# srihari-humbarwadi/retinanet-tensorflow2.x

Hardware: AMD Instinct MI355X
Metric: images/sec train, ResNet50-640 RetinaNet data-parallel step (encode + fwd + loss + bwd + clip + all-reduce + SGD/EMA); inference images/s under `infer` (higher is better)
Workload: dtype bf16; 1 GPU; ResNet50-640x640 bf16 training, 32 images/GPU (BASELINE configs[2] shard: global batch 32), resnet_initial frozen, single GPU; global_batch=32, parallelism=dp1, rccl_ranks=1, comm=torch, syncbn_messages=0

## Files before the change

### include/rnet_hip.h

```cpp
#ifndef RNET_HIP_H_
#define RNET_HIP_H_

#include <stddef.h>
#include <stdint.h>

#ifdef __cplusplus
extern "C" {
#endif
#if defined(__GNUC__)
#pragma GCC visibility push(default)
#endif

typedef enum {
  RN_OK = 0,
  RN_EINVAL = -1,
  RN_ENOMEM = -2,
  RN_EHIP = -3,
  RN_ECOMM = -4,
  RN_EUNSUPPORTED = -5
} rn_status;

enum { RN_DT_F32 = 0, RN_DT_BF16 = 1 };
enum { RN_ACT_NONE = 0, RN_ACT_RELU = 1, RN_ACT_RELU6 = 2, RN_ACT_SWISH = 3 };

// ... 67 lines not shown
  int32_t wgrad_target_blocks;
  int32_t ablate;
  int32_t splitk_target_blocks;
} rn_launch_opts;

typedef struct rn_handle rn_handle;
int rn_create(int device_id, rn_handle** out);
int rn_destroy(rn_handle* h);
int rn_handle_device(const rn_handle* h);
int rn_handle_num_cus(const rn_handle* h);
int rn_handle_set_launch_opts(rn_handle* h, const rn_launch_opts* opts);
int rn_handle_get_launch_opts(const rn_handle* h, rn_launch_opts* opts);
int rn_handle_comm_init(rn_handle* h, int slot, const void* unique_id , int rank, int world);
void* rn_handle_comm(const rn_handle* h, int slot);
int rn_handle_comm_destroy(rn_handle* h, int slot);

#define RN_CONV_MAX_SEGMENTS 10

typedef struct {
  const void* x;
  const void* w;
  void* y;
  const float* scale;
  const float* shift;
  const void* residual;
  int32_t N, H, W, Cin, pix_stride, Ho, Wo, Cout;
  float* bn_partial;
  const float* bias;
  int32_t w_terms;
  int32_t w_pair;
  const void* bn_bwd_y;
  const float* bn_bwd_fwd;
} rn_conv_segment;

typedef struct {
  int32_t R, S, stride_h, stride_w, pad_top, pad_left;
  int32_t act;
  int32_t out_dtype;
  int32_t num_segments;
  rn_conv_segment seg[RN_CONV_MAX_SEGMENTS];
  rn_launch_opts opts;
  void* splitk_ws;
  int64_t splitk_ws_bytes;
} rn_conv_problem;

int rn_conv2d_nhwc_fwd(const rn_conv_problem* problem , void* stream);
size_t rn_conv_splitk_workspace_bytes(const rn_conv_problem* problem );
size_t rn_conv_splitk_workspace_max_bytes(void);

int rn_conv_cout_pad(int Cout);
int rn_conv_tile_rows(const rn_conv_problem* problem);
int rn_conv_bn_row_blocks(const rn_conv_problem* problem, int segment);
int rn_conv_kernel_id(const rn_conv_problem* problem);
int rn_conv_cin_pad(int Cin);
int rn_pack_conv_weight(const float* w_hwio, int R, int S, int Cin, int Cout, int Cin_pad, void* w_packed,
                        void* stream);
int rn_pack_conv_weight_split(const float* w, int layout_ohwi, int R, int S, int Cin, int Cout, int Cin_pad, int terms,
                              void* w_packed, void* stream);
int rn_conv_pair_rows(int Cout);
int rn_pack_conv_weight_pair(const float* w, int layout_ohwi, int R, int S, int Cin, int Cout, int Cin_pad,
                             void* w_packed, void* stream);
int rn_pack_conv_weight_ohwi(const float* w_ohwi, int R, int S, int Cin, int Cout, int Cin_pad, void* w_packed,
                             void* stream);
int rn_pack_stem_weight(const float* w_hwio, int Cout, void* w_packed, void* stream);
int rn_stem_padded_width(int W);
int rn_pack_stem_input(const float* images, int N, int H, int W, void* packed, void* stream);
int rn_pack_stem_weight_rs(const float* w_hwio, int R, int S, int Cout, void* w_packed, void* stream);
int rn_pack_image_nhwc4(const float* images, int N, int H, int W, int pad_top, int pad_left, int Hp, int Wp,
                        void* packed, void* stream);

typedef struct {
  const void* x;
  const void* dy;
  int32_t N, H, W, Cin, Ho, Wo, Cout;
  int32_t dy_pix_stride;
  int32_t x_pix_stride;
} rn_wgrad_segment;

typedef struct {
  int32_t R, S, stride_h, stride_w, pad_top, pad_left;
  int32_t num_segments;
  rn_wgrad_segment seg[RN_CONV_MAX_SEGMENTS];
  rn_launch_opts opts;
} rn_wgrad_problem;

size_t rn_wgrad_workspace_bytes(const rn_wgrad_problem* problem );
int rn_wgrad_kernel_id(const rn_wgrad_problem* problem );
int rn_conv2d_nhwc_wgrad(const rn_wgrad_problem* problem , float* dw, float beta, void* workspace,
                         size_t workspace_bytes, void* stream);
size_t rn_wgrad_group_workspace_bytes(const rn_wgrad_problem* const* problems , int n);
int rn_wgrad_group_fused(const rn_wgrad_problem* const* problems , int n);
int rn_conv2d_nhwc_wgrad_group(const rn_wgrad_problem* const* problems , int n, float* const* dws ,
                               float beta, void* workspace, size_t workspace_bytes, void* stream);

int rn_pack_conv_weight_dgrad(const float* w_ohwi, int R, int S, int Cin, int Cout, int Cout_pad, void* w_packed,
                              void* stream);
#define RN_DGRAD_PACK_MAX 64
typedef struct {
  const float* w_ohwi;
  void* w_packed;
  int32_t R, S, Cin, Cout, Cout_pad;
  int32_t pad_;
} rn_dgrad_pack;
int rn_pack_conv_weight_dgrad_batch(const rn_dgrad_pack* items , int n, void* stream);
int rn_cast_pad_f32_to_bf16(const float* x, void* y, int64_t P, int C, int Cpad, void* stream);
int rn_reduce_rows_f32(const float* src, int rows, int64_t row_stride, int n, float add, float* dst, void* stream);
// ... 188 lines not shown
```

### retinanet-tensorflow2.x_amd/csrc/rn_conv_dev.h

```cpp
#ifndef RN_CONV_DEV_H_
#define RN_CONV_DEV_H_
#include "rn_common.h"

typedef rn_h16 bf16x8_t __attribute__((ext_vector_type(8)));
typedef float f32x16_t __attribute__((ext_vector_type(16)));

#define CONV_THREADS 256

struct ConvSegDev {
  const uint16_t* x;
  const uint16_t* w;
  void* y;
  const float* scale;
  const float* shift;
  const uint16_t* residual;
  float* bn_partial;
  const float* bias;
  const uint16_t* bn_y;
  const float* bn_fwd;
  int N, H, W, Cin, pix_stride, Ho, Wo, Cout;
  int M, tile_begin, n_tiles, CinP;
  int cwrap, halo_pitch;
  int pair_cout, rows;
};


struct ConvArgs {
  int R, S, sh, sw, pt, pl, act, nseg, total_tiles, pad_;
  int split_f, split_s, vtotal, pad2_;
  float* ws;
  ConvSegDev seg[RN_CONV_MAX_SEGMENTS];
};

#define RN_SPLITK_HEADER_BYTES 16384
#define RN_SPLITK_SLOT_BYTES (256 * 256 * 4)

template <int BK>
__device__ __forceinline__ int lds_swz(int row) {
  constexpr int SLOTS = BK / 8;
  constexpr int RPB = 256 / (BK * 2);
  return (row / RPB) % SLOTS;
}
template <int BK>
__device__ __forceinline__ int lds_slot_off(int row, int slot) {
  return (row * (BK / 8) + (slot ^ lds_swz<BK>(row))) * 16;
}

typedef __attribute__((address_space(3))) void lds_void_t;

__device__ __forceinline__ void dma16(__amdgpu_buffer_rsrc_t rsrc, char* lds_wave_base, unsigned voff) {
  __builtin_amdgcn_raw_ptr_buffer_load_lds(rsrc, (lds_void_t*)lds_wave_base, 16, (int)voff, 0, 0, 0);
}

#define RN_OOB 0x80000000u


int rn_launch_conv128(const ConvArgs& a, int BN, int BK, bool f32, bool split, hipStream_t st);
int rn_launch_conv_big(const ConvArgs& a, bool out_f32, const rn_launch_opts& opts, hipStream_t st);
int rn_launch_conv_halo(const ConvArgs& a, bool out_f32, const rn_launch_opts& opts, hipStream_t st, int wm = 2);
int rn_conv_halo_patch_pixels(int N, int H, int W, int pitch, int BM = 256);
int rn_conv_halo_pitch(int W);
int rn_conv_halo_capacity(int BM = 256);
#endif
```

### retinanet-tensorflow2.x_amd/csrc/rn_conv_dispatch.hip

```cpp
#include <algorithm>
#include <map>
#include <mutex>
#include <tuple>

#include "rn_conv_dev.h"

extern "C" int rn_conv_cout_pad(int Cout) { return Cout <= 64 ? 64 : (int)rn_align_up((size_t)Cout, 128); }
extern "C" int rn_conv_cin_pad(int Cin) { return Cin <= 32 ? 32 : (int)rn_align_up((size_t)Cin, 64); }
extern "C" int rn_conv_pair_rows(int Cout) { return Cout > 0 ? 128 * ((Cout + 63) / 64) : 0; }

struct ConvPlanSeg {
  int cols, cols_pad;
  int terms, cin_pad;
  long long M;
  int n_tiles, tile_begin;
  int bn_row_blocks;
};

struct ConvPlan {
  int kid;
  int BM, BN;
  int BK;
  int bal_rows;
  bool deal;
  bool fast_div;
  int order[RN_CONV_MAX_SEGMENTS];
  long long total_tiles;
  int min_depth;
  int split_parts;
  long long ws_bytes;
  ConvPlanSeg seg[RN_CONV_MAX_SEGMENTS];
};

static long long seg_tiles(const ConvPlanSeg& s, int rows, int width) { return rn_cdiv(s.M, rows) * rn_cdiv(s.cols_pad, width); }
static long long conv_tiles(const ConvPlan& pl, int nseg, int rows, int width) {
  long long t = 0;
  for (int i = 0; i < nseg; ++i) t += seg_tiles(pl.seg[i], rows, width);
  return t;
}

static bool conv_halo_fits(const rn_conv_problem* p, int BM) {
  if (p->opts.conv_no_halo) return false;
  if (p->R != 3 || p->S != 3 || p->stride_h != 1 || p->stride_w != 1 || p->pad_top != 1 || p->pad_left != 1)
    return false;
  static std::mutex mu;
  static std::map<std::tuple<int, int, int, int>, int> patch_px;
  for (int i = 0; i < p->num_segments; ++i) {
    const rn_conv_segment& s = p->seg[i];
    if (s.Ho != s.H || s.Wo != s.W || s.Cin % 32 != 0) return false;
    if ((long long)s.N * s.H * s.W >= (1ll << 22)) return false;
    std::lock_guard<std::mutex> lock(mu);
    const auto key = std::make_tuple(s.N, s.H, s.W, BM);
    auto it = patch_px.find(key);
    if (it == patch_px.end()) it = patch_px.emplace(key, rn_conv_halo_patch_pixels(s.N, s.H, s.W, rn_conv_halo_pitch(s.W), BM)).first;
    if (it->second > rn_conv_halo_capacity(BM)) return false;
  }
  return true;
}

static int splitk_parts(int total, int min_chunks, int G0, long long* bytes) {
  const int L = total % G0;
  if (bytes) *bytes = 0;
  if (L == 0 || L > 511 || min_chunks < 8) return 1;
  int S = G0 / L;
  if (S > min_chunks / 4) S = min_chunks / 4;
  if (S > 4) S = 4;
  if (S < 2) return 1;
  if (bytes) *bytes = RN_SPLITK_HEADER_BYTES + (long long)L * S * RN_SPLITK_SLOT_BYTES;
  return S;
}

static void rn_splitk_plan(ConvArgs& a, int min_chunks, void* ws, long long ws_bytes, const rn_launch_opts& opts) {
  const int total = a.total_tiles;
  a.split_f = total; a.split_s = 1; a.vtotal = total; a.pad2_ = 0; a.ws = nullptr;
  const int G0 = rn_persistent_grid(0x7fffffff, rn_num_cus(), opts);
  const int L = total % G0;
  int S = ws ? splitk_parts(total, min_chunks, G0, nullptr) : 1;
  while (S >= 2 && RN_SPLITK_HEADER_BYTES + (long long)L * S * RN_SPLITK_SLOT_BYTES > ws_bytes) --S;
  if (S < 2) return;
  a.split_f = total - L; a.split_s = S; a.vtotal = L * S; a.ws = (float*)ws;
}

extern "C" size_t rn_conv_splitk_workspace_max_bytes(void) { return RN_SPLITK_HEADER_BYTES + 256ull * RN_SPLITK_SLOT_BYTES; }

static int conv_big_balanced_rows(const rn_conv_problem* p, const ConvPlanSeg& s) {
  if (p->num_segments != 1 || p->R != 1 || p->S != 1 || p->stride_h != 1 || p->stride_w != 1) return 0;
  if (p->opts.conv_tile || p->opts.conv_big_min_tiles || p->opts.max_workgroups || p->splitk_ws) return 0;
  if (s.terms * s.cin_pad > 512) return 0;
  const int n_tiles = (int)rn_cdiv(s.cols_pad, 256);
  const int G = rn_persistent_grid(0x7fffffff, rn_num_cus(), p->opts);
  const long long T = seg_tiles(s, 256, 256);
  if (T <= 0 || G <= 0) return 0;
  const long long rounds = rn_cdiv(T, G);
  const long long m_tiles = rounds * G / n_tiles;
  if (m_tiles < 1) return 0;
  long long rows = rn_cdiv(s.M, m_tiles);
  rows = (rows + 3) / 4 * 4;
  if (rows < 64 || rows > 236) return 0;
  return (int)rows;
}

#define RN_SPLIT128_MIN_STEPS 4
static int conv128_split_parts(const rn_launch_opts& opts, long long tiles, int ksteps, int BN, long long ws_bytes) {
  if (opts.conv_tile == 1 || tiles < 1 || tiles > 4096) return 1;
  const int target = opts.splitk_target_blocks > 0 ? opts.splitk_target_blocks : rn_num_cus() * 3 / 4;
  int S = target / (int)tiles;
  if (S > ksteps / RN_SPLIT128_MIN_STEPS) S = ksteps / RN_SPLIT128_MIN_STEPS;
  if (S > 8) S = 8;
  const long long slot = 128ll * BN * 4;
  while (S >= 2 && RN_SPLITK_HEADER_BYTES + tiles * S * slot > ws_bytes) --S;
  return S >= 2 ? S : 1;
}

static bool conv_plan(const rn_conv_problem* p, bool assume_ws, ConvPlan& pl) {
  if (!p || p->num_segments < 1 || p->num_segments > RN_CONV_MAX_SEGMENTS) return false;
  const int nseg = p->num_segments;
  const rn_launch_opts& o = p->opts;

  bool all_wide = true, all_128 = true, all_128s_or_64 = true, one_col = true;
  bool epi_ok = true;
  long long dmin = 1ll << 60, dmax = 0;
  pl.min_depth = 0x7fffffff;
  pl.fast_div = true;
  for (int i = 0; i < nseg; ++i) {
    const rn_conv_segment& s = p->seg[i];
    ConvPlanSeg& d = pl.seg[i];
    d.cols = s.w_pair ? rn_conv_pair_rows(s.Cout) : s.Cout;
    d.cols_pad = rn_conv_cout_pad(d.cols);
    d.terms = s.w_terms > 1 ? s.w_terms : 1;
    d.cin_pad = rn_conv_cin_pad(s.Cin);
    d.M = (long long)s.N * s.Ho * s.Wo;
    all_wide = all_wide && d.cols_pad >= 256;
    all_128 = all_128 && d.cols_pad == 128;
    all_128s_or_64 = all_128s_or_64 && (d.cols_pad % 128 == 0 || d.cols_pad == 64);
    one_col = one_col && d.cols_pad <= 256;
    epi_ok = epi_ok && s.Cout % (p->out_dtype == RN_DT_F32 && s.w_pair ? 4 : 8) == 0 && !(s.bias && s.residual);
    const int depth = d.terms * d.cin_pad;
    pl.min_depth = depth < pl.min_depth ? depth : pl.min_depth;
    const long long depth_all = (long long)p->R * p->S * d.cin_pad * d.terms;
    dmin = depth_all < dmin ? depth_all : dmin;
    dmax = depth_all > dmax ? depth_all : dmax;
    pl.fast_div = pl.fast_div && d.M < (1 << 22);
  }
  const int cin0 = pl.seg[0].cin_pad;
  pl.BK = (cin0 % 64 != 0 || (long long)p->R * p->S * cin0 <= 256) ? 32 : 64;

  const bool use_big = o.conv_tile != 1 && o.conv_tile != 3 && all_wide && epi_ok &&
                       (o.conv_tile == 2 || conv_tiles(pl, nseg, 256, 256) >= (o.conv_big_min_tiles > 0 ? o.conv_big_min_tiles : 192));
  if (use_big) {
    if (!conv_halo_fits(p, 256)) pl.kid = 1;
    else pl.kid = (o.conv_tile == 0 && o.conv_big_min_tiles == 0 && conv_halo_fits(p, 512)) ? 3 : 2;
  } else {
    const bool halo512 = o.conv_tile != 1 && !o.conv_no_halo && (o.conv_tile == 3 ? all_128s_or_64 : all_128) && epi_ok &&
                         (o.conv_tile >= 2 || conv_tiles(pl, nseg, 512, 128) >= (o.conv_big_min_tiles > 0 ? o.conv_big_min_tiles : 128)) &&
                         conv_halo_fits(p, 512);
    pl.kid = halo512 ? 3 : 0;
  }

  pl.bal_rows = 0;
  if (pl.kid == 0) {
    pl.BM = 128;
    pl.BN = pl.seg[0].cols_pad <= 64 ? 64 : 128;
    if (pl.BN == 128 && o.conv_tile != 1 && 2 * conv_tiles(pl, nseg, 128, 128) <= rn_num_cus()) pl.BN = 64;
  } else if (pl.kid == 3) {
    pl.BM = 512; pl.BN = 128;
  } else {
    pl.BM = 256; pl.BN = 256;
    if (pl.kid == 1) pl.bal_rows = conv_big_balanced_rows(p, pl.seg[0]);
  }

  for (int i = 0; i < nseg; ++i) pl.order[i] = i;
  pl.deal = pl.kid == 1 && nseg > 1 && one_col && dmax >= 2 * dmin;
  if (pl.deal)
    std::stable_sort(pl.order, pl.order + nseg, [&](int x, int y) {
      return pl.seg[x].cin_pad * pl.seg[x].terms > pl.seg[y].cin_pad * pl.seg[y].terms;
    });
  const int rows = pl.bal_rows ? pl.bal_rows : pl.BM;
  pl.total_tiles = 0;
  for (int ii = 0; ii < nseg; ++ii) {
    ConvPlanSeg& d = pl.seg[pl.order[ii]];
    d.n_tiles = (int)rn_cdiv(d.cols_pad, pl.BN);
    d.tile_begin = (int)pl.total_tiles;
    d.bn_row_blocks = (int)(pl.bal_rows ? 2 * rn_cdiv(d.M, rows) : (rows / 128) * rn_cdiv(d.M, rows));
    pl.total_tiles += seg_tiles(d, rows, pl.BN);
  }

  pl.split_parts = 1;
  pl.ws_bytes = 0;
  if (pl.kid == 0) {
    if (p->splitk_ws || assume_ws) {
      const long long avail = p->splitk_ws ? p->splitk_ws_bytes : (long long)rn_conv_splitk_workspace_max_bytes();
      pl.split_parts = conv128_split_parts(o, pl.total_tiles, p->R * p->S * (pl.min_depth / pl.BK), pl.BN, avail);
    }
    if (pl.split_parts >= 2) pl.ws_bytes = RN_SPLITK_HEADER_BYTES + pl.total_tiles * pl.split_parts * 128 * pl.BN * 4;
  } else if (pl.kid == 2) {
    splitk_parts((int)pl.total_tiles, pl.min_depth / 32, rn_persistent_grid(0x7fffffff, rn_num_cus(), o), &pl.ws_bytes);
  }
  return true;
}

extern "C" size_t rn_conv_splitk_workspace_bytes(const rn_conv_problem* p) {
  ConvPlan pl;
  return conv_plan(p, true, pl) ? (size_t)pl.ws_bytes : 0;
}

extern "C" int rn_conv_kernel_id(const rn_conv_problem* p) {
  ConvPlan pl;
  return conv_plan(p, false, pl) ? pl.kid : -1;
}

extern "C" int rn_conv_bn_row_blocks(const rn_conv_problem* p, int segment) {
  ConvPlan pl;
  if (!conv_plan(p, false, pl) || segment < 0 || segment >= p->num_segments) return 0;
  return pl.seg[segment].bn_row_blocks;
}

extern "C" int rn_conv_tile_rows(const rn_conv_problem* p) {
  ConvPlan pl;
  return conv_plan(p, false, pl) ? pl.BM : 0;
}

static int conv_validate(const rn_conv_problem* p, const ConvPlan& pl) {
  RN_CHECK_ARG(p->R >= 1 && p->S >= 1 && p->R * p->S <= 32, "rn_conv2d_nhwc_fwd: R*S=%d > 32", p->R * p->S);
  RN_CHECK_ARG(p->stride_h >= 1 && p->stride_w >= 1, "rn_conv2d_nhwc_fwd: bad stride");
  RN_CHECK_ARG(p->out_dtype == RN_DT_BF16 || p->out_dtype == RN_DT_F32, "rn_conv2d_nhwc_fwd: bad out_dtype");
  if (const int orc = rn_validate_launch_opts(p->opts, "rn_conv2d_nhwc_fwd")) return orc;
  for (int ii = 0; ii < p->num_segments; ++ii) {
    const int i = pl.order[ii];
    const rn_conv_segment& s = p->seg[i];
    RN_CHECK_ARG(s.x && s.w && s.y, "rn_conv2d_nhwc_fwd: segment %d has a null tensor", i);
    RN_CHECK_ARG(s.N > 0 && s.H > 0 && s.W > 0 && s.Ho > 0 && s.Wo > 0 && s.Cout > 0 && s.Cin > 0,
                 "rn_conv2d_nhwc_fwd: segment %d bad shape", i);
    RN_CHECK_ARG(s.Cin % 8 == 0 && pl.seg[i].cin_pad % pl.BK == 0,
                 "rn_conv2d_nhwc_fwd: segment %d Cin=%d must be a multiple of 8 (K step %d)", i, s.Cin, pl.BK);
    RN_CHECK_ARG(s.pix_stride % 4 == 0 && s.pix_stride > 0,
                 "rn_conv2d_nhwc_fwd: segment %d pix_stride=%d must be a positive multiple of 4", i, s.pix_stride);
    RN_CHECK_ARG(s.Cout % 4 == 0, "rn_conv2d_nhwc_fwd: segment %d Cout=%d not a multiple of 4", i, s.Cout);
    RN_CHECK_ARG((pl.seg[i].cols_pad <= 64) == (pl.seg[0].cols_pad <= 64), "rn_conv2d_nhwc_fwd: segments mix Cout tile widths");
    RN_CHECK_ARG(!s.w_pair || (pl.kid != 0 && p->out_dtype == RN_DT_F32 && s.w_terms <= 1 && !s.scale && !s.shift &&
                               !s.residual && !s.bn_partial),
                 "rn_conv2d_nhwc_fwd: segment %d: w_pair needs an f32 launch without scale / shift / residual that the 256- / "
                 "512-row kernels take (rn_conv_kernel_id() != 0)", i);
    RN_CHECK_ARG(((uintptr_t)s.x | (uintptr_t)s.w | (uintptr_t)s.y | (uintptr_t)s.residual) % 16 == 0,
                 "rn_conv2d_nhwc_fwd: segment %d tensors must be 16-byte aligned", i);
    RN_CHECK_ARG(pl.seg[i].M < (1ll << 31) && (long long)s.N * s.H * s.W * s.pix_stride * 2 < (1ll << 31),
                 "rn_conv2d_nhwc_fwd: segment %d input exceeds the 2 GiB buffer-addressing limit", i);
    if (s.bn_bwd_y) {
      RN_CHECK_ARG(s.bn_partial && s.bn_bwd_fwd && p->out_dtype == RN_DT_BF16 && !s.scale && !s.shift && !s.bias &&
                       !s.residual && p->act == RN_ACT_NONE && s.Cout % 8 == 0 && (uintptr_t)s.bn_bwd_y % 16 == 0,
                   "rn_conv2d_nhwc_fwd: segment %d: bn_bwd_y needs bn_partial + bn_bwd_fwd on a plain bf16 launch", i);
    }
    RN_CHECK_ARG((s.bn_bwd_y != nullptr) == (p->seg[0].bn_bwd_y != nullptr),
                 "rn_conv2d_nhwc_fwd: bn_bwd_y must be set on all segments or none");
    RN_CHECK_ARG(pl.seg[i].terms <= 3, "rn_conv2d_nhwc_fwd: segment %d w_terms=%d (1..3)", i, s.w_terms);
  }
  RN_CHECK_ARG(p->splitk_ws == nullptr || ((uintptr_t)p->splitk_ws % 16 == 0 && p->splitk_ws_bytes >= 0),
               "rn_conv2d_nhwc_fwd: splitk_ws must be 16-byte aligned");
  return RN_OK;
}

extern "C" int rn_conv2d_nhwc_fwd(const rn_conv_problem* p, void* stream) {
  RN_CHECK_ARG(p != nullptr, "rn_conv2d_nhwc_fwd: null problem");
  RN_CHECK_ARG(p->num_segments >= 1 && p->num_segments <= RN_CONV_MAX_SEGMENTS,
               "rn_conv2d_nhwc_fwd: num_segments=%d", p->num_segments);
  ConvPlan pl;
  conv_plan(p, false, pl);
  if (const int rc = conv_validate(p, pl)) return rc;

  ConvArgs a;
  a.R = p->R; a.S = p->S; a.sh = p->stride_h; a.sw = p->stride_w; a.pt = p->pad_top; a.pl = p->pad_left;
  a.act = p->act; a.nseg = p->num_segments;
  a.total_tiles = (int)pl.total_tiles;
  a.pad_ = pl.kid <= 1 ? (pl.fast_div ? 1 : 0) | (pl.deal ? 2 : 0) : 0;
  a.split_f = a.vtotal = a.total_tiles; a.split_s = 1; a.pad2_ = 0; a.ws = nullptr;
  for (int ii = 0; ii < p->num_segments; ++ii) {
    const rn_conv_segment& s = p->seg[pl.order[ii]];
    const ConvPlanSeg& ps = pl.seg[pl.order[ii]];
    ConvSegDev& d = a.seg[ii];
    d.x = (const uint16_t*)s.x; d.w = (const uint16_t*)s.w; d.y = s.y;
    d.scale = s.scale; d.shift = s.shift; d.residual = (const uint16_t*)s.residual;
    d.bn_partial = s.bn_partial;
    d.bn_y = (const uint16_t*)s.bn_bwd_y;
    d.bn_fwd = s.bn_bwd_fwd;
    d.bias = s.bias;
    d.N = s.N; d.H = s.H; d.W = s.W; d.Cin = s.Cin; d.pix_stride = s.pix_stride;
    d.Ho = s.Ho; d.Wo = s.Wo; d.Cout = ps.cols;
    d.pair_cout = s.w_pair ? s.Cout : 0;
    d.rows = pl.bal_rows;
    d.M = (int)ps.M;
    d.tile_begin = ps.tile_begin;
    d.n_tiles = ps.n_tiles;
    d.cwrap = ps.cin_pad;
    d.CinP = ps.terms * ps.cin_pad;
    d.halo_pitch = s.W + 1;
  }

  hipStream_t st = (hipStream_t)stream;
  const bool f32 = p->out_dtype == RN_DT_F32;
  switch (pl.kid) {
    case 3: return rn_launch_conv_halo(a, f32, p->opts, st, 4);
    case 2:
      rn_splitk_plan(a, pl.min_depth / 32, p->splitk_ws, p->splitk_ws_bytes, p->opts);
      return rn_launch_conv_halo(a, f32, p->opts, st);
    case 1: return rn_launch_conv_big(a, f32, p->opts, st);
  }
  if (pl.split_parts >= 2) {
    a.split_s = pl.split_parts; a.vtotal = a.total_tiles * pl.split_parts; a.ws = (float*)p->splitk_ws;
  }
  return rn_launch_conv128(a, pl.BN, pl.BK, f32, pl.split_parts >= 2, st);
}
```

### retinanet-tensorflow2.x_amd/retinanet/_C.py

```python
from __future__ import annotations

import ctypes
import logging
import os
from ctypes import (POINTER, Structure, c_char_p, c_float, c_int, c_int32, c_int64, c_longlong, c_size_t, c_uint32,
                    c_uint64, c_void_p)

_HERE = os.path.dirname(os.path.abspath(__file__))
LIB_PATH = os.environ.get("RNET_HIP_LIB") or os.path.join(_HERE, "librnet_hip.so")
LIB_PATH_F16 = os.environ.get("RNET_HIP_LIB_F16") or os.path.join(_HERE, "librnet_hip_f16.so")

RN_DT_F32, RN_DT_BF16 = 0, 1
RN_OK, RN_EINVAL, RN_ENOMEM, RN_EHIP, RN_ECOMM, RN_EUNSUPPORTED = 0, -1, -2, -3, -4, -5
RN_ACT_NONE, RN_ACT_RELU, RN_ACT_RELU6, RN_ACT_SWISH = 0, 1, 2, 3
RN_CONV_MAX_SEGMENTS = 10
ABI_VERSION = 8
PRED_W_TERMS = int(os.environ.get("RNET_PRED_W_TERMS", "2"))
ACT_IDS = {None: RN_ACT_NONE, "none": RN_ACT_NONE, "relu": RN_ACT_RELU, "relu6": RN_ACT_RELU6,
           "swish": RN_ACT_SWISH}


class RnetError(RuntimeError):
    pass

# ... 76 lines not shown
                ("dres", c_void_p), ("sums", c_void_p), ("fwd", c_void_p), ("bsums", c_void_p),
                ("gamma", c_void_p), ("beta", c_void_p), ("moving_mean", c_void_p), ("moving_var", c_void_p),
                ("dgamma", c_void_p), ("dbeta", c_void_p), ("P", c_int64), ("C", c_int32),
                ("dres_accumulate", c_int32), ("sample_scale", c_void_p), ("rows_per_sample", c_int64),
                ("ext_chunks", c_int32), ("ext_chunks_bwd", c_int32), ("act_mask", c_void_p),
                ("dy_colsum_partial", c_void_p)]


class BnProblem(Structure):
    _fields_ = [("num_segments", c_int32), ("act", c_int32), ("bessel", c_int32), ("eps", c_float),
                ("momentum", c_float), ("count_scale", c_float), ("seg", BnSegment * RN_CONV_MAX_SEGMENTS)]


_PP = POINTER(c_void_p)
_SIGNATURES = {
    "rn_last_error": (c_char_p, []),
    "rn_abi_version": (c_int, []),
    "rn_storage_dtype": (c_int, []),
    "rn_device_ok": (c_int, []),
    "rn_anchors_generate": (c_int, [c_void_p, c_int64, c_int, c_int, c_int, c_int, POINTER(c_float),
                                    POINTER(c_float), c_int, POINTER(c_float), c_int, POINTER(c_int64),
                                    c_void_p]),
    "rn_match_workspace_bytes": (c_size_t, [c_int, c_int]),
    "rn_anchor_match_encode": (c_int, [c_void_p, c_int64, c_void_p, c_void_p, c_void_p, c_int, c_int, c_float,
                                       c_float, POINTER(c_float), c_void_p, c_void_p, c_void_p, c_void_p,
                                       c_void_p, c_size_t, c_void_p]),
    "rn_loss_workspace_bytes": (c_size_t, [c_int, c_int64, c_int]),
    "rn_retinanet_loss_fwd_bwd": (c_int, [_PP, _PP, _PP, _PP, POINTER(c_int64), c_int, c_int, c_int, c_void_p,
                                          c_void_p, c_void_p, c_float, c_float, c_float, c_float, c_float,
                                          c_float, c_float, c_void_p, c_void_p, c_size_t, c_void_p]),
    "rn_retinanet_loss_fwd_bwd_bf16": (c_int, [_PP, _PP, _PP, _PP, c_int, c_int, c_int, POINTER(c_int64), c_int, c_int,
                                               c_int, c_void_p, c_void_p, c_void_p, c_float, c_float, c_float, c_float,
                                               c_float, c_float, c_float, c_void_p, c_void_p, c_size_t, c_void_p]),
    "rn_decode_boxes": (c_int, [_PP, POINTER(c_int64), c_int, c_int, c_void_p, POINTER(c_float), c_float,
                                c_float, c_void_p, c_void_p]),
    "rn_sigmoid_scores": (c_int, [_PP, POINTER(c_int64), c_int, c_int, c_int, c_void_p, c_void_p]),
    "rn_topk_workspace_bytes": (c_size_t, [c_int, c_int64, c_int]),
    "rn_topk_per_class": (c_int, [c_void_p, c_int, c_int64, c_int, c_int, c_void_p, c_void_p, c_void_p,
                                  c_size_t, c_void_p]),
    "rn_detect_workspace_bytes": (c_size_t, [c_int, c_int64, c_int, c_int]),
    "rn_detect_per_class": (c_int, [_PP, POINTER(c_int64), c_int, c_int, c_int, c_void_p, c_int, c_float,
                                    c_float, c_float, c_int, c_void_p, c_void_p, c_void_p, c_void_p, c_void_p,
                                    c_size_t, c_void_p]),
    "rn_nms_workspace_bytes": (c_size_t, [c_int, c_int, c_int, c_int]),
    "rn_nms_per_class": (c_int, [c_void_p, c_void_p, c_int, c_int, c_int, c_float, c_float, c_float, c_int,
                                 c_void_p, c_void_p, c_void_p, c_void_p, c_void_p, c_void_p, c_size_t, c_void_p]),
    "rn_rowmax_argmax": (c_int, [c_void_p, c_int64, c_int, c_void_p, c_void_p, c_void_p]),
    "rn_conv2d_nhwc_fwd": (c_int, [POINTER(ConvProblem), c_void_p]),
    "rn_conv_cout_pad": (c_int, [c_int]),
    "rn_conv_tile_rows": (c_int, [POINTER(ConvProblem)]),
    "rn_conv_bn_row_blocks": (c_int, [POINTER(ConvProblem), c_int]),
    "rn_probe_spin": (c_int, [c_int, c_void_p]),
    "rn_conv_kernel_id": (c_int, [POINTER(ConvProblem)]),
    "rn_conv_splitk_workspace_bytes": (c_size_t, [POINTER(ConvProblem)]),
    "rn_conv_splitk_workspace_max_bytes": (c_size_t, []),
    "rn_conv_cin_pad": (c_int, [c_int]),
    "rn_depthwise_conv2d_nhwc_fwd": (c_int, [POINTER(DwProblem), c_void_p]),
    "rn_pack_depthwise_weight": (c_int, [c_void_p, c_int, c_int, c_void_p, c_void_p]),
    "rn_pack_depthwise_weight_flip": (c_int, [c_void_p, c_int, c_int, c_void_p, c_void_p]),
    "rn_depthwise_wgrad_workspace_bytes": (c_size_t, [POINTER(DwProblem)]),
    "rn_depthwise_conv2d_nhwc_wgrad": (c_int, [POINTER(DwProblem), c_void_p, c_void_p, c_size_t, c_void_p]),
    "rn_squeeze_excite_fwd": (c_int, [c_void_p, c_void_p, c_int, c_int, c_int, c_void_p, c_void_p, c_void_p, c_void_p,
                                      c_int, c_void_p, c_size_t, c_void_p]),
    "rn_squeeze_excite_bwd": (c_int, [c_void_p, c_void_p, c_void_p, c_int, c_int, c_int, c_void_p, c_void_p, c_int,
                                      c_void_p, c_void_p, c_void_p, c_void_p, c_void_p, c_void_p, c_size_t, c_void_p]),
    "rn_coco_accumulate": (c_int, [c_void_p, c_void_p, c_void_p, c_void_p, c_float, c_float, c_void_p, c_int, c_int, c_int,
                                   c_int, c_void_p, c_void_p, c_void_p]),
    "rn_pack_conv_weight_ohwi": (c_int, [c_void_p, c_int, c_int, c_int, c_int, c_int, c_void_p, c_void_p]),
    "rn_se_workspace_bytes": (c_size_t, [c_int, c_int]),
    "rn_squeeze_excite_inplace": (c_int, [c_void_p, c_int, c_int, c_int, c_void_p, c_void_p, c_void_p, c_void_p,
                                          c_int, c_void_p, c_size_t, c_void_p]),
    "rn_pack_conv_weight": (c_int, [c_void_p, c_int, c_int, c_int, c_int, c_int, c_void_p, c_void_p]),
    "rn_conv_pair_rows": (c_int, [c_int]),
    "rn_pack_conv_weight_pair": (c_int, [c_void_p, c_int, c_int, c_int, c_int, c_int, c_int, c_void_p, c_void_p]),
    "rn_pack_conv_weight_split": (c_int, [c_void_p, c_int, c_int, c_int, c_int, c_int, c_int, c_int, c_void_p,
                                          c_void_p]),
    "rn_pack_stem_weight": (c_int, [c_void_p, c_int, c_void_p, c_void_p]),
    "rn_stem_padded_width": (c_int, [c_int]),
    "rn_pack_stem_input": (c_int, [c_void_p, c_int, c_int, c_int, c_void_p, c_void_p]),
    "rn_pack_stem_weight_rs": (c_int, [c_void_p, c_int, c_int, c_int, c_void_p, c_void_p]),
    "rn_pack_image_nhwc4": (c_int, [c_void_p, c_int, c_int, c_int, c_int, c_int, c_int, c_int, c_void_p, c_void_p]),
    "rn_wgrad_workspace_bytes": (c_size_t, [POINTER(WgradProblem)]),
    "rn_wgrad_kernel_id": (c_int, [POINTER(WgradProblem)]),
    "rn_conv2d_nhwc_wgrad": (c_int, [POINTER(WgradProblem), c_void_p, c_float, c_void_p, c_size_t, c_void_p]),
    "rn_wgrad_group_workspace_bytes": (c_size_t, [POINTER(POINTER(WgradProblem)), c_int]),
    "rn_wgrad_group_fused": (c_int, [POINTER(POINTER(WgradProblem)), c_int]),
    "rn_conv2d_nhwc_wgrad_group": (c_int, [POINTER(POINTER(WgradProblem)), c_int, _PP, c_float, c_void_p, c_size_t,
                                           c_void_p]),
    "rn_pack_conv_weight_dgrad": (c_int, [c_void_p, c_int, c_int, c_int, c_int, c_int, c_void_p, c_void_p]),
    "rn_pack_conv_weight_dgrad_batch": (c_int, [POINTER(DgradPack), c_int, c_void_p]),
    "rn_cast_pad_f32_to_bf16": (c_int, [c_void_p, c_void_p, c_int64, c_int, c_int, c_void_p]),
    "rn_reduce_rows_f32": (c_int, [c_void_p, c_int, c_int64, c_int, c_float, c_void_p, c_void_p]),
    "rn_upsample_zero2x": (c_int, [c_void_p, c_void_p, c_int, c_int, c_int, c_int, c_int, c_int, c_void_p]),
    "rn_scatter_add2x": (c_int, [c_void_p, c_void_p, c_int, c_int, c_int, c_int, c_int, c_int, c_int, c_void_p]),
    "rn_depth_to_space2x": (c_int, [c_void_p, c_void_p, c_int, c_int, c_int, c_int, c_int, c_void_p]),
    "rn_cast_f32_to_bf16": (c_int, [c_void_p, c_void_p, c_int64, c_void_p]),
    "rn_act_bwd": (c_int, [c_void_p, c_void_p, c_void_p, c_int64, c_int, c_void_p]),
    "rn_bn_workspace_bytes": (c_size_t, [POINTER(BnProblem)]),
    "rn_bn_workspace_init": (c_int, [POINTER(BnProblem), c_void_p, c_size_t, c_void_p]),
    "rn_bn_partial_offset_bytes": (c_size_t, [POINTER(BnProblem), c_int]),
    "rn_bn_bwd_partial_offset_bytes": (c_size_t, [POINTER(BnProblem), c_int]),
    "rn_bn_stats": (c_int, [POINTER(BnProblem), c_void_p, c_size_t, c_void_p]),
    "rn_bn_stats_finalize": (c_int, [POINTER(BnProblem), c_void_p, c_size_t, c_void_p]),
    "rn_bn_finalize": (c_int, [POINTER(BnProblem), c_void_p]),
    "rn_bn_apply": (c_int, [POINTER(BnProblem), c_void_p]),
    "rn_bn_bwd_reduce": (c_int, [POINTER(BnProblem), c_void_p, c_size_t, c_void_p]),
# ... 261 lines not shown
```

### retinanet-tensorflow2.x_amd/retinanet/model/train_engine.py

```python
from __future__ import annotations

import ctypes
import os
from typing import NamedTuple

import numpy as np
import torch

from retinanet import _C
from .bottleneck import Bottleneck64, fused_blocks
from .forward import (FoldedConvs, conv_launch_name, conv_problem, dw_problem, half_activations, maxpool_step, split_by_depth,
                      stem_input, stem_pool_partner, stem_pool_step, stem_problem, tensor_readers, topdown_step)

_DT = {"bf16": torch.bfloat16, "f32": torch.float32}
_SEG_DTYPE = np.dtype([("offset", "<i8"), ("size", "<i8"), ("wd", "<i4"), ("bb", "<i4"), ("nb", "<i4"),
                       ("pad", "<i4"), ("bf", "<i8")])


def _hwio_to_ohwi(w):
    return w.permute(3, 0, 1, 2).contiguous()


def _ohwi_to_hwio(w):
    return w.permute(1, 2, 3, 0).contiguous()
# ... 442 lines not shown
                need.add(op["out"])
                for i in [op["inp"]] + ([op["residual"]] if op.get("residual") else []):
                    if self.requires.get(i):
                        need.add(i)
            elif op["op"] in ("maxpool",) and self.requires.get(op["out"]):
                need.add(op["out"])
                if self.requires.get(op["inp"]):
                    need.add(op["inp"])
            elif op["op"] == "topdown":
                for n in op["ins"] + op["outs"]:
                    if self.requires.get(n):
                        need.add(n)
        for n in need:
            H, W, C, _ = self.tensors[n]
            self.grad[n] = torch.zeros((B, H, W, C), dtype=self.h16, device=dev)
        for n, t in self.bal_out.items():
            self.grad["bal:" + n] = torch.zeros_like(t)
        self.bn_state = {}
        for op in self.ops:
            if op["op"] in ("conv", "stem", "dwconv") and self._bn_trainable(op):
                bn = op["bn"]
                self.bn_state[bn] = {"mm": self.model.variables[bn + "/moving_mean"].to(dev, torch.float32).clone(),
                                     "mv": self.model.variables[bn + "/moving_variance"].to(dev, torch.float32).clone()}

    def _fold_frozen(self):
        for op in self.ops:
            if op["op"] in ("conv", "stem") and not self._conv_trainable(op) and op["out"] not in self._bneck_skip:
                self.folded.load(self.model.variables, op)
        for fb in self.bneck.values():
            fb.load(self.model.variables, self.eps)

    def _conv_meta(self, p):
        osz = 4 if p.out_dtype == _C.RN_DT_F32 else 2
        dom = True
        for i in range(p.num_segments):
            s = p.seg[i]
            dom = dom and s.Cout > 64 and s.Cin % 64 == 0 and p.out_dtype == _C.RN_DT_BF16
        if id(p) in self._algo:
            flops, byts = self._algo[id(p)]
        else:
            flops = byts = 0
            for i in range(p.num_segments):
                s = p.seg[i]
                flops += 2 * s.N * s.Ho * s.Wo * p.R * p.S * s.Cin * s.Cout
                byts += 2 * s.N * s.H * s.W * s.pix_stride + osz * s.N * s.Ho * s.Wo * s.Cout + 2 * p.R * p.S * s.Cin * s.Cout
                if s.residual:
                    byts += 2 * s.N * s.Ho * s.Wo * s.Cout
        variant = None
        kid = self.lib.rn_conv_kernel_id(ctypes.byref(p))
        has_res = any(p.seg[i].residual for i in range(p.num_segments))
        bnb = bool(p.seg[0].bn_bwd_y)
        tmpl = (f"<{'true' if p.out_dtype == _C.RN_DT_F32 else 'false'}, {'true' if has_res else 'false'}, "
                f"{'true' if bnb else 'false'}>")
        if kid == 2:
            variant = "conv_halo_kernel" + tmpl[:-1] + ", false, 2> (256x256x32, 3x3 halo patch)"
        elif kid == 3:
            variant = "conv_halo_kernel" + tmpl[:-1] + ", false, 4> (512x128x32, 3x3 halo patch)"
        elif kid == 1:
            variant = "conv_big_kernel" + tmpl + " (256x256x32)"
        elif dom:
            variant = "conv_fwd_kernel<128,128,64,bf16>"
        return flops, byts, variant

    def _timed(self, launch, *sinks):
        cur = torch.cuda.current_stream(self.dev)
        e0, e1 = torch.cuda.Event(enable_timing=True), torch.cuda.Event(enable_timing=True)
        e0.record(cur)
        launch()
        e1.record(cur)
        for lst, row in sinks:
            if lst is not None:
                lst.append((e0, e1) + row)

    def _launch_conv(self, p, st, what):
        prof, lprof = self.conv_profile, self.layer_profile
        if prof is not None or lprof is not None:
            flops, byts, variant = self._conv_meta(p)
            if variant or lprof is not None:
                lrow = None
                if lprof is not None:
                    kid = self.lib.rn_conv_kernel_id(ctypes.byref(p))
                    kname = variant or ("conv_fwd_kernel (128-row tiles)" if kid == 0 else f"kernel id {kid}")
                    lrow = (self._launch_names.get(id(p), what), flops, byts, kname)
                self._timed(lambda: _C.check(self.lib.rn_conv2d_nhwc_fwd(ctypes.byref(p), st), what),
                            (prof if variant else None, (flops, byts, variant)), (lprof, lrow))
                return
        _C.check(self.lib.rn_conv2d_nhwc_fwd(ctypes.byref(p), st), what)

    def _weight_ptr(self, cname):
        if cname in self.fwd_pack_of:
            return self.fwd_pack_of[cname].data_ptr()
        if cname in self.split_pack_of:
            return self.split_pack_of[cname].data_ptr()
        return self.Pbf.data_ptr() + 2 * self.bf_off[cname]

    def _f32_terms(self, layer):
        if _C.PRED_W_TERMS <= 1:
            return 1
        return _C.PRED_W_TERMS if self.folded.w_pair(layer) else self.wide_pred_terms

    def _group_ops(self, kind, grp):
        return [o for o in self.ops if o["op"] == kind and o.get("group") == grp]

    def _conv_problem(self, ops, dst_of, raw_mode):
        p = conv_problem(self.g, ops, self.B, self.launch_opts, self.splitk_ws, lambda o: self._src(o["inp"]), dst_of,
                         self.folded.pixel_pair, _C.RN_ACT_NONE if raw_mode else None)
        for i, op in enumerate(ops):
# ... 1172 lines not shown
```

Before: 1129 images/s.

## Add weight-stationary streaming kernel for 1x1 stride-1 bf16 convolutions

Adds a new persistent 1x1 convolution kernel that loads a whole Cout slab of weights into LDS once per block, then streams row ranges of activations through MFMA with register double-buffering. It fuses residual add and BN partial statistics into the epilogue. Dispatch routes qualifying single-segment 1x1 bf16 convs with no activation or scale/shift to it. The aim is to cut repeated weight reloads and tile overhead in the bottleneck expand/project convs, at the cost of large LDS use per block and lower occupancy.

Result: no change. 1129 images/s (median of 3 runs) (+0.1%).

```diff
diff --git a/include/rnet_hip.h b/include/rnet_hip.h
--- a/include/rnet_hip.h
+++ b/include/rnet_hip.h
@@ -143,6 +143,7 @@
 int rn_conv_tile_rows(const rn_conv_problem* problem);
 int rn_conv_bn_row_blocks(const rn_conv_problem* problem, int segment);
 int rn_conv_kernel_id(const rn_conv_problem* problem);
+int rn_conv_launch_kernel_id(const rn_conv_problem* problem);
 int rn_conv_cin_pad(int Cin);
 int rn_pack_conv_weight(const float* w_hwio, int R, int S, int Cin, int Cout, int Cin_pad, void* w_packed,
                         void* stream);
diff --git a/retinanet-tensorflow2.x_amd/csrc/rn_conv_dev.h b/retinanet-tensorflow2.x_amd/csrc/rn_conv_dev.h
--- a/retinanet-tensorflow2.x_amd/csrc/rn_conv_dev.h
+++ b/retinanet-tensorflow2.x_amd/csrc/rn_conv_dev.h
@@ -57,6 +57,7 @@
 
 int rn_launch_conv128(const ConvArgs& a, int BN, int BK, bool f32, bool split, hipStream_t st);
 int rn_launch_conv_big(const ConvArgs& a, bool out_f32, const rn_launch_opts& opts, hipStream_t st);
+int rn_launch_conv_stream(const ConvArgs& a, hipStream_t st);
 int rn_launch_conv_halo(const ConvArgs& a, bool out_f32, const rn_launch_opts& opts, hipStream_t st, int wm = 2);
 int rn_conv_halo_patch_pixels(int N, int H, int W, int pitch, int BM = 256);
 int rn_conv_halo_pitch(int W);
diff --git a/retinanet-tensorflow2.x_amd/csrc/rn_conv_dispatch.hip b/retinanet-tensorflow2.x_amd/csrc/rn_conv_dispatch.hip
--- a/retinanet-tensorflow2.x_amd/csrc/rn_conv_dispatch.hip
+++ b/retinanet-tensorflow2.x_amd/csrc/rn_conv_dispatch.hip
@@ -29,6 +29,8 @@
   int min_depth;
   int split_parts;
   long long ws_bytes;
+  int stream;
+  int st_slabs, st_ranges;
   ConvPlanSeg seg[RN_CONV_MAX_SEGMENTS];
 };
 
@@ -110,6 +112,18 @@
   const long long slot = 128ll * BN * 4;
   while (S >= 2 && RN_SPLITK_HEADER_BYTES + tiles * S * slot > ws_bytes) --S;
   return S >= 2 ? S : 1;
+}
+
+static int conv_stream_slab(const rn_conv_problem* p) {
+  if (p->num_segments != 1 || p->R != 1 || p->S != 1 || p->stride_h != 1 || p->stride_w != 1 || p->pad_top != 0 ||
+      p->pad_left != 0 || p->out_dtype != RN_DT_BF16 || p->act != RN_ACT_NONE)
+    return 0;
+  if (p->opts.conv_tile || p->opts.conv_big_min_tiles) return 0;
+  const rn_conv_segment& s = p->seg[0];
+  if (s.Cin != 64 && s.Cin != 128 && s.Cin != 256 && s.Cin != 512) return 0;
+  if (s.Cout < 256 || s.Cout % 8 != 0 || s.pix_stride % 8 != 0 || s.Ho != s.H || s.Wo != s.W) return 0;
+  if (s.w_terms > 1 || s.w_pair || s.scale || s.shift || s.bias || s.bn_bwd_y || (s.residual && s.bn_partial)) return 0;
+  return s.Cin <= 256 ? 256 : 128;
 }
 
 static bool conv_plan(const rn_conv_problem* p, bool assume_ws, ConvPlan& pl) {
@@ -196,6 +210,17 @@
   } else if (pl.kid == 2) {
     splitk_parts((int)pl.total_tiles, pl.min_depth / 32, rn_persistent_grid(0x7fffffff, rn_num_cus(), o), &pl.ws_bytes);
   }
+
+  pl.stream = conv_stream_slab(p);
+  pl.st_slabs = pl.st_ranges = 0;
+  if (pl.stream) {
+    const long long units = rn_cdiv(pl.seg[0].M, 128);
+    pl.st_slabs = (int)rn_cdiv(pl.seg[0].cols, pl.stream);
+    long long ranges = rn_persistent_grid(0x7fffffff, rn_num_cus(), o) / pl.st_slabs;
+    if (ranges > units) ranges = units;
+    if (ranges >= 8) ranges -= ranges % 8;
+    pl.st_ranges = ranges < 1 ? 1 : (int)ranges;
+  }
   return true;
 }
 
@@ -207,6 +232,11 @@
 extern "C" int rn_conv_kernel_id(const rn_conv_problem* p) {
   ConvPlan pl;
   return conv_plan(p, false, pl) ? pl.kid : -1;
+}
+
+extern "C" int rn_conv_launch_kernel_id(const rn_conv_problem* p) {
+  ConvPlan pl;
+  return conv_plan(p, false, pl) ? (pl.stream ? 4 : pl.kid) : -1;
 }
 
 extern "C" int rn_conv_bn_row_blocks(const rn_conv_problem* p, int segment) {
@@ -297,6 +327,10 @@
 
   hipStream_t st = (hipStream_t)stream;
   const bool f32 = p->out_dtype == RN_DT_F32;
+  if (pl.stream) {
+    a.total_tiles = pl.st_ranges; a.split_s = pl.st_slabs; a.vtotal = pl.seg[0].bn_row_blocks;
+    return rn_launch_conv_stream(a, st);
+  }
   switch (pl.kid) {
     case 3: return rn_launch_conv_halo(a, f32, p->opts, st, 4);
     case 2:
diff --git a/retinanet-tensorflow2.x_amd/csrc/rn_conv_stream.hip b/retinanet-tensorflow2.x_amd/csrc/rn_conv_stream.hip
--- /dev/null
+++ b/retinanet-tensorflow2.x_amd/csrc/rn_conv_stream.hip
@@ -0,0 +1,248 @@
+#include "rn_conv_big_epi.h"
+
+namespace {
+
+constexpr int ST_NW = 8, ST_PATCH = 4096;
+
+template <int KS, bool HAS_RES>
+__global__ void __launch_bounds__(512) conv1x1_stream_kernel(const ConvArgs args) {
+  extern __shared__ __attribute__((aligned(16))) char smem[];
+  constexpr int K = KS * 16;
+  constexpr int BN = K <= 256 ? 256 : 128;
+  constexpr int NP = BN / 128;
+  constexpr int W_BYTES = BN * K * 2;
+  const ConvSegDev& sg = args.seg[0];
+  const int tid = threadIdx.x;
+  const int lane = tid & 63;
+  const int wave = __builtin_amdgcn_readfirstlane(tid >> 6);
+  const int M = sg.M, Cout = sg.Cout;
+  const int nrange = args.total_tiles, nslab = args.split_s;
+
+  int range, slab;
+  {
+    const int b = blockIdx.x;
+    if (nrange >= 8) {
+      const int j = b >> 3;
+      const int q = j / nslab;
+      slab = j - q * nslab;
+      range = (b & 7) + 8 * q;
+    } else {
+      range = b / nslab;
+      slab = b - range * nslab;
+    }
+  }
+  const int n0 = slab * BN;
+  const int units = (M + 127) >> 7;
+  const int u_begin = (int)((long long)range * units / nrange), u_end = (int)((long long)(range + 1) * units / nrange);
+  const int npass = (Cout - n0 + 127) / 128 < NP ? (Cout - n0 + 127) / 128 : NP;
+
+  {
+    const int rows_pad = Cout <= 64 ? 64 : ((Cout + 127) / 128) * 128;
+    const __amdgpu_buffer_rsrc_t rs_w =
+        __builtin_amdgcn_make_buffer_rsrc((void*)sg.w, 0, (int)((long long)rows_pad * K * 2), 0x00020000);
+    const int fr = lane & 31, fh = lane >> 5;
+#pragma unroll 4
+    for (int f = wave; f < (BN / 32) * KS; f += ST_NW) {
+      const int tile = f / KS, s = f - tile * KS;
+      const int row = n0 + tile * 32 + fr;
+      const unsigned voff = row < rows_pad ? (unsigned)((row * K + s * 16 + fh * 8) * 2) : RN_OOB;
+      dma16(rs_w, smem + f * 1024, voff);
+    }
+    asm volatile("s_waitcnt vmcnt(0)" ::: "memory");
+    __syncthreads();
+  }
+  char* const patch = smem + W_BYTES + wave * ST_PATCH;
+
+  const int nu = u_end - u_begin;
+  const int my_units = wave < nu ? (nu - wave + ST_NW - 1) / ST_NW : 0;
+  const int nitems = my_units * npass * 4;
+  const __amdgpu_buffer_rsrc_t rs_x = __builtin_amdgcn_make_buffer_rsrc(
+      (void*)sg.x, 0, (int)((long long)sg.N * sg.H * sg.W * sg.pix_stride * 2), 0x00020000);
+  const int fr = lane & 31, fh = lane >> 5;
+  const int rrow = lane >> 3, ru = lane & 7;
+  const int row_bytes_x = sg.pix_stride * 2;
+  auto x_off = [&](int q) -> unsigned {
+    const int blk = q & 3, r = q >> 2;
+    const int ui = npass == 2 ? r >> 1 : r;
+    const int m = (u_begin + wave + ST_NW * ui) * 128 + blk * 32 + fr;
+    return (q < nitems && m < M) ? (unsigned)(m * row_bytes_x + fh * 16) : RN_OOB;
+  };
+  constexpr int KH = KS < 16 ? KS : 16, NH = KS / KH;
+  bf16x8_t xq[KH];
+  {
+    const unsigned v0 = x_off(0);
+#pragma unroll
+    for (int s = 0; s < KH; ++s)
+      xq[s] = __builtin_bit_cast(bf16x8_t, __builtin_amdgcn_raw_buffer_load_b128(rs_x, v0, s * 32, 0));
+  }
+  const bool stats = !HAS_RES && sg.bn_partial != nullptr;
+  float st0[2][8], st1[2][8];
+#pragma unroll
+  for (int j = 0; j < 2; ++j)
+#pragma unroll
+    for (int q = 0; q < 8; ++q) st0[j][q] = st1[j][q] = 0.0f;
+  float one = 1.0f, zero = 0.0f;
+  asm volatile("" : "+v"(one), "+v"(zero));
+  const long long row_bytes = (long long)Cout * 2;
+
+#pragma unroll 1
+  for (int q = 0; q < nitems; ++q) {
+    const int blk = q & 3, r = q >> 2;
+    const int pass = npass == 2 ? r & 1 : 0;
+    const int unit = u_begin + wave + ST_NW * (npass == 2 ? r >> 1 : r);
+    const int m0 = unit * 128 + blk * 32;
+    const int nc0 = n0 + pass * 128;
+    const unsigned vcur = x_off(q), vnext = x_off(q + 1);
+
+    uint4 rv[HAS_RES ? 2 : 1][HAS_RES ? 4 : 1];
+    if (HAS_RES) {
+#pragma unroll
+      for (int jr = 0; jr < 2; ++jr)
+#pragma unroll
+        for (int p4 = 0; p4 < 4; ++p4) {
+          const int m = m0 + p4 * 8 + rrow, nr = nc0 + jr * 64 + ru * 8;
+          rv[HAS_RES ? jr : 0][HAS_RES ? p4 : 0] = make_uint4(0u, 0u, 0u, 0u);
+          if (m < M && nr < Cout) rv[HAS_RES ? jr : 0][HAS_RES ? p4 : 0] = *(const uint4*)(sg.residual + (long long)m * Cout + nr);
+        }
+    }
+
+    f32x16_t acc[4];
+#pragma unroll
+    for (int t = 0; t < 4; ++t)
+#pragma unroll
+      for (int e = 0; e < 16; ++e) acc[t][e] = 0.0f;
+    const char* const wl = smem + (pass * 4 * KS) * 1024 + lane * 16;
+    bf16x8_t wf[2][4];
+#pragma unroll
+    for (int t = 0; t < 4; ++t) wf[0][t] = *(const bf16x8_t*)(wl + (t * KS) * 1024);
+#pragma unroll
+    for (int ks = 0; ks < KS; ++ks) {
+      const int hf = ks / KH, s = ks % KH;
+      if (ks + 1 < KS) {
+#pragma unroll
+        for (int t = 0; t < 4; ++t) wf[(ks + 1) & 1][t] = *(const bf16x8_t*)(wl + (t * KS + ks + 1) * 1024);
+      }
+      __builtin_amdgcn_sched_barrier(0);
+#pragma unroll
+      for (int t = 0; t < 4; ++t) acc[t] = RN_MFMA_32x32x16(wf[ks & 1][t], xq[s], acc[t], 0, 0, 0);
+      if (hf + 1 < NH)
+        xq[s] = __builtin_bit_cast(bf16x8_t, __builtin_amdgcn_raw_buffer_load_b128(rs_x, vcur, ((hf + 1) * KH + s) * 32, 0));
+      else
+        xq[s] = __builtin_bit_cast(bf16x8_t, __builtin_amdgcn_raw_buffer_load_b128(rs_x, vnext, s * 32, 0));
+      __builtin_amdgcn_sched_barrier(0);
+    }
+
+#pragma unroll
+    for (int jr = 0; jr < 2; ++jr) {
+      const int nr = nc0 + jr * 64 + ru * 8;
+      const bool nok = nr < Cout;
+#pragma unroll
+      for (int j = 0; j < 2; ++j)
+#pragma unroll
+        for (int g = 0; g < 4; ++g) {
+          const int nl = j * 32 + g * 8 + fh * 4;
+          const f32x16_t& a = acc[jr * 2 + j];
+          uint2 pk;
+          pk.x = pack2(a[g * 4 + 0], a[g * 4 + 1]);
+          pk.y = pack2(a[g * 4 + 2], a[g * 4 + 3]);
+          *(uint2*)(patch + fr * 128 + (((nl >> 3) ^ (fr & 7)) << 4) + ((((nl >> 2) ^ (fr >> 3)) & 1) << 3)) = pk;
+        }
+      uint4 vb[4];
+#pragma unroll
+      for (int p4 = 0; p4 < 4; ++p4) {
+        const int row = p4 * 8 + rrow;
+        const uint4 t = *(const uint4*)(patch + row * 128 + ((ru ^ (row & 7)) << 4));
+        vb[p4] = (p4 & 1) ? make_uint4(t.z, t.w, t.x, t.y) : t;
+      }
+#pragma unroll
+      for (int p4 = 0; p4 < 4; ++p4) {
+        const int m = m0 + p4 * 8 + rrow;
+        if (m < M && nok) {
+          uint4 ov = vb[p4];
+          if (HAS_RES) {
+            const uint4 v = vb[p4], r4 = rv[HAS_RES ? jr : 0][HAS_RES ? p4 : 0];
+            float f[8] = {bf_lo(v.x), bf_hi(v.x), bf_lo(v.y), bf_hi(v.y), bf_lo(v.z), bf_hi(v.z), bf_lo(v.w), bf_hi(v.w)};
+            const float rr[8] = {bf_lo(r4.x), bf_hi(r4.x), bf_lo(r4.y), bf_hi(r4.y),
+                                 bf_lo(r4.z), bf_hi(r4.z), bf_lo(r4.w), bf_hi(r4.w)};
+#pragma unroll
+            for (int e = 0; e < 8; ++e) f[e] = (f[e] * one + zero) + rr[e];
+            ov.x = pack2(f[0], f[1]); ov.y = pack2(f[2], f[3]); ov.z = pack2(f[4], f[5]); ov.w = pack2(f[6], f[7]);
+          }
+          *(uint4*)((char*)sg.y + (long long)m * row_bytes + (long long)nr * 2) = ov;
+          if (!HAS_RES && stats) {
+            const float w[8] = {bf_lo(ov.x), bf_hi(ov.x), bf_lo(ov.y), bf_hi(ov.y),
+                                bf_lo(ov.z), bf_hi(ov.z), bf_lo(ov.w), bf_hi(ov.w)};
+#pragma unroll
+            for (int e = 0; e < 8; ++e) { st0[jr][e] += w[e]; st1[jr][e] += w[e] * w[e]; }
+          }
+        }
+      }
+    }
+
+    if (!HAS_RES && stats && blk == 3) {
+#pragma unroll
+      for (int jr = 0; jr < 2; ++jr) {
+#pragma unroll
+        for (int e = 0; e < 8; ++e) {
+#pragma unroll
+          for (int o = 8; o < 64; o <<= 1) {
+            st0[jr][e] += __shfl_xor(st0[jr][e], o, 64);
+            st1[jr][e] += __shfl_xor(st1[jr][e], o, 64);
+          }
+        }
+        const int nr = nc0 + jr * 64 + ru * 8;
+        if (rrow == 0 && nr < Cout) {
+          float* dst = sg.bn_partial + (long long)unit * 2 * Cout + nr;
+          *(float4*)(dst) = make_float4(st0[jr][0], st0[jr][1], st0[jr][2], st0[jr][3]);
+          *(float4*)(dst + 4) = make_float4(st0[jr][4], st0[jr][5], st0[jr][6], st0[jr][7]);
+          *(float4*)(dst + Cout) = make_float4(st1[jr][0], st1[jr][1], st1[jr][2], st1[jr][3]);
+          *(float4*)(dst + Cout + 4) = make_float4(st1[jr][4], st1[jr][5], st1[jr][6], st1[jr][7]);
+        }
+#pragma unroll
+        for (int e = 0; e < 8; ++e) st0[jr][e] = st1[jr][e] = 0.0f;
+      }
+    }
+  }
+
+  if (!HAS_RES && stats && range == nrange - 1) {
+    const int extra = args.vtotal - units;
+    const int c4 = ((Cout - n0 < BN ? Cout - n0 : BN) + 3) / 4;
+    for (int i = tid; i < extra * 2 * c4; i += blockDim.x) {
+      const int rw = i / c4, c = i - rw * c4;
+      *(float4*)(sg.bn_partial + ((long long)units * 2 + rw) * Cout + n0 + c * 4) = make_float4(0.f, 0.f, 0.f, 0.f);
+    }
+  }
+}
+
+template <int KS>
+int stream_launch(const ConvArgs& a, bool has_res, dim3 grid, hipStream_t st) {
+  constexpr int K = KS * 16, BN = K <= 256 ? 256 : 128;
+  constexpr int LDS = BN * K * 2 + ST_NW * ST_PATCH;
+  static unsigned long long attr_set = 0;
+  if (RN_ATTRS_NEEDED(attr_set)) {
+    RN_CHECK_HIP(hipFuncSetAttribute((const void*)conv1x1_stream_kernel<KS, false>,
+                                     hipFuncAttributeMaxDynamicSharedMemorySize, LDS));
+    RN_CHECK_HIP(hipFuncSetAttribute((const void*)conv1x1_stream_kernel<KS, true>,
+                                     hipFuncAttributeMaxDynamicSharedMemorySize, LDS));
+    RN_ATTRS_DONE(attr_set);
+  }
+  if (has_res) hipLaunchKernelGGL((conv1x1_stream_kernel<KS, true>), grid, dim3(512), LDS, st, a);
+  else hipLaunchKernelGGL((conv1x1_stream_kernel<KS, false>), grid, dim3(512), LDS, st, a);
+  RN_CHECK_LAUNCH();
+  return RN_OK;
+}
+
+}
+
+int rn_launch_conv_stream(const ConvArgs& a, hipStream_t st) {
+  const dim3 grid((unsigned)(a.total_tiles * a.split_s));
+  const bool has_res = a.seg[0].residual != nullptr;
+  switch (a.seg[0].Cin) {
+    case 64: return stream_launch<4>(a, has_res, grid, st);
+    case 128: return stream_launch<8>(a, has_res, grid, st);
+    case 256: return stream_launch<16>(a, has_res, grid, st);
+    case 512: return stream_launch<32>(a, has_res, grid, st);
+  }
+  rn_set_error("rn_launch_conv_stream: Cin=%d (64 | 128 | 256 | 512)", a.seg[0].Cin);
+  return RN_EINVAL;
+}
diff --git a/retinanet-tensorflow2.x_amd/retinanet/_C.py b/retinanet-tensorflow2.x_amd/retinanet/_C.py
--- a/retinanet-tensorflow2.x_amd/retinanet/_C.py
+++ b/retinanet-tensorflow2.x_amd/retinanet/_C.py
@@ -152,6 +152,7 @@
     "rn_conv_bn_row_blocks": (c_int, [POINTER(ConvProblem), c_int]),
     "rn_probe_spin": (c_int, [c_int, c_void_p]),
     "rn_conv_kernel_id": (c_int, [POINTER(ConvProblem)]),
+    "rn_conv_launch_kernel_id": (c_int, [POINTER(ConvProblem)]),
     "rn_conv_splitk_workspace_bytes": (c_size_t, [POINTER(ConvProblem)]),
     "rn_conv_splitk_workspace_max_bytes": (c_size_t, []),
     "rn_conv_cin_pad": (c_int, [c_int]),
diff --git a/retinanet-tensorflow2.x_amd/retinanet/model/train_engine.py b/retinanet-tensorflow2.x_amd/retinanet/model/train_engine.py
--- a/retinanet-tensorflow2.x_amd/retinanet/model/train_engine.py
+++ b/retinanet-tensorflow2.x_amd/retinanet/model/train_engine.py
@@ -518,7 +518,10 @@
         bnb = bool(p.seg[0].bn_bwd_y)
         tmpl = (f"<{'true' if p.out_dtype == _C.RN_DT_F32 else 'false'}, {'true' if has_res else 'false'}, "
                 f"{'true' if bnb else 'false'}>")
-        if kid == 2:
+        if self.lib.rn_conv_launch_kernel_id(ctypes.byref(p)) == 4:
+            variant = (f"conv1x1_stream_kernel<{p.seg[0].Cin // 16}, {'true' if has_res else 'false'}> "
+                       f"(weights in LDS, {256 if p.seg[0].Cin <= 256 else 128}-channel slabs)")
+        elif kid == 2:
             variant = "conv_halo_kernel" + tmpl[:-1] + ", false, 2> (256x256x32, 3x3 halo patch)"
         elif kid == 3:
             variant = "conv_halo_kernel" + tmpl[:-1] + ", false, 4> (512x128x32, 3x3 halo patch)"
```
